# zuds-survey/zuds-pipeline

Hardware: AMD Instinct MI355X
Metric: Mpix/s resample->coadd->subtract, 3072x3072 frames (higher is better)
Workload: dtype f32; 1 GPU; configs[1]+[2]: 32x 3072x3072 TPV frames/GPU, mesh background + weight rescale + Lanczos-3 resample + WEIGHTED coadd (+ AND mask coadd, int16 masks); then 1 science frame/GPU: align ref, hotpants 3x3 regions x 10x10 stamps, r=10, ko=4, subtract; frames_per_gpu=32, size=3072, mask_dtype=int16, combine=WEIGHTED, subtract=True

## Files before the change

### zuds-pipeline_amd/csrc/hotpants.hip

```cpp
#include "hp_dev.h"
#include <sched.h>
#include "chol_diag.h"

static __device__ __forceinline__ void hp_zero_words(int* __restrict__ zero0, int nzero0, int* __restrict__ zero1, int nzero1) {
    if (blockIdx.x != 0) return;
    if (zero0) for (int k = threadIdx.x; k < nzero0; k += blockDim.x) zero0[k] = 0;
    if (zero1) for (int k = threadIdx.x; k < nzero1; k += blockDim.x) zero1[k] = 0;
}
__global__ void k_hp_valid(const float* __restrict__ sci, const float* __restrict__ ref,
                           const uint8_t* __restrict__ bpm, int64_t n, float il, float iu,
                           float tl, float tu, uint8_t* __restrict__ bad,
                           const double* __restrict__ lim, double nsig,
                           int* __restrict__ zero0 = nullptr, int nzero0 = 0,
                           int* __restrict__ zero1 = nullptr, int nzero1 = 0) {
    int64_t p = (int64_t)blockIdx.x * blockDim.x + threadIdx.x;
    hp_zero_words(zero0, nzero0, zero1, nzero1);
    if (lim) {
        il = (float)(lim[0] - nsig * lim[1]);
        tl = (float)(lim[3] - nsig * lim[4]);
    }
    if (p >= n) return;
    float s = sci[p], t = ref[p];
    bool ok = (s == s) && (t == t) && fabsf(s) < 3e38f && fabsf(t) < 3e38f;
    ok = ok && s >= il && s <= iu && t >= tl && t <= tu;
// ... 367 lines not shown
#define GR_PITCH 34

#define GR_SPLIT 8
template <int NT, int R0, int C0, int R1, int C1, int R2, int C2>
static __device__ __forceinline__ void hp_gram_ktile(const double* L, int li, int lk, double4_t (&acc)[3]) {
#pragma unroll
    for (int kk = 0; kk < GR_KT / 4; ++kk) {
        const double* Lk = L + li * GR_PITCH + 4 * kk + lk;
        acc[0] = __builtin_amdgcn_mfma_f64_16x16x4f64(Lk[16 * R0 * GR_PITCH], Lk[16 * C0 * GR_PITCH], acc[0], 0, 0, 0);
        if (NT > 1) acc[1] = __builtin_amdgcn_mfma_f64_16x16x4f64(Lk[16 * R1 * GR_PITCH], Lk[16 * C1 * GR_PITCH], acc[1], 0, 0, 0);
        if (NT > 2) acc[2] = __builtin_amdgcn_mfma_f64_16x16x4f64(Lk[16 * R2 * GR_PITCH], Lk[16 * C2 * GR_PITCH], acc[2], 0, 0, 0);
    }
}
template <int R, int C>
static __device__ __forceinline__ void hp_gram_store(double* Gc, int li, int lk, const double4_t& a) {
#pragma unroll
    for (int rg = 0; rg < 4; ++rg) {
        Gc[(size_t)(16 * R + lk + 4 * rg) * HP_MAXX + 16 * C + li] = a[rg];
        if (R != C) Gc[(size_t)(16 * C + li) * HP_MAXX + 16 * R + lk + 4 * rg] = a[rg];
    }
}
#define GR_DEAL(sel, F) \
    switch (sel) { \
        case 0: F(3, 3, 0, 3, 1, 3, 2) break; \
        case 1: F(3, 2, 0, 2, 1, 2, 2) break; \
        case 2: F(2, 1, 0, 1, 1, 0, 0) break; \
        default: F(2, 0, 0, 3, 3, 0, 0) break; \
    }
static __device__ __forceinline__ void hp_gram_body(const hp_plan& P, const double* __restrict__ X,
                                                 const int* __restrict__ need,
                                                 const int* __restrict__ active,
                                                 double* __restrict__ Gp, const int* __restrict__ guard,
                                                 const int* __restrict__ list) {
    if (guard && *guard == 0) return;
    __shared__ double L[HP_MAXX * GR_PITCH];
    const int tid = threadIdx.x;
    const int ncl = list ? list[0] : (int)gridDim.x;
#pragma unroll 1
    for (int ci = blockIdx.x; ci < ncl; ci += gridDim.x) {
    const int cell = list ? list[1 + ci] : ci;
    __syncthreads();
    if (!need[cell] || active[cell] < 0) continue;
    const double* Xc = X + (size_t)cell * P.nX * P.npixp;
    const int wave = tid >> 6, lane = tid & 63;
    const int li = lane & 15, lk = lane >> 4;
    const int sel = __builtin_amdgcn_readfirstlane((wave + blockIdx.x + blockIdx.y) & 3);
    const int ntile = P.npixp / GR_KT;
    const int per = (ntile + GR_SPLIT - 1) / GR_SPLIT;
    const int kbeg = blockIdx.y * per * GR_KT, kend = min((int)(blockIdx.y + 1) * per, ntile) * GR_KT;
    double4_t acc[3];
#pragma unroll
    for (int c = 0; c < 3; ++c) acc[c] = (double4_t){0.0, 0.0, 0.0, 0.0};
    constexpr int GR_LD = HP_MAXX * GR_KT / 256;
    double nxt[GR_LD];
    auto fetch = [&](int k0) {
#pragma unroll
        for (int q = 0; q < GR_LD; ++q) {
            const int e = tid + 256 * q, row = e >> 5, col = e & 31;
            nxt[q] = row < P.nX ? Xc[(size_t)row * P.npixp + k0 + col] : 0.0;
        }
    };
    if (kbeg < kend) fetch(kbeg);
    for (int k0 = kbeg; k0 < kend; k0 += GR_KT) {
        __syncthreads();
#pragma unroll
        for (int q = 0; q < GR_LD; ++q) {
            const int e = tid + 256 * q, row = e >> 5, col = e & 31;
            L[row * GR_PITCH + col] = nxt[q];
        }
        __syncthreads();
        if (k0 + GR_KT < kend) fetch(k0 + GR_KT);
#define GR_STEP(NT, R0, C0, R1, C1, R2, C2) hp_gram_ktile<NT, R0, C0, R1, C1, R2, C2>(L, li, lk, acc);
        GR_DEAL(sel, GR_STEP)
#undef GR_STEP
    }
    double* Gc = Gp + ((size_t)cell * GR_SPLIT + blockIdx.y) * HP_MAXX * HP_MAXX;
#define GR_OUT(NT, R0, C0, R1, C1, R2, C2) { \
        hp_gram_store<R0, C0>(Gc, li, lk, acc[0]); \
        if (NT > 1) hp_gram_store<R1, C1>(Gc, li, lk, acc[1]); \
        if (NT > 2) hp_gram_store<R2, C2>(Gc, li, lk, acc[2]); }
    GR_DEAL(sel, GR_OUT)
#undef GR_OUT
    }
}
#undef GR_DEAL

#define GS_THREADS 1024
static __device__ __forceinline__ void hp_gram_sum_body(const double* __restrict__ Gp,
                                                     const int* __restrict__ need,
                                                     const int* __restrict__ active,
                                                     double* __restrict__ G, const int* __restrict__ guard,
                                                     double* __restrict__ Gold, const int* __restrict__ list) {
    if (guard && *guard == 0) return;
    const int ncl = list ? list[0] : (int)gridDim.x;
    constexpr int NE = HP_MAXX * HP_MAXX / GS_THREADS;
#pragma unroll 1
    for (int ci = blockIdx.x; ci < ncl; ci += gridDim.x) {
        const int cell = list ? list[1 + ci] : ci;
        if (!need[cell] || active[cell] < 0) continue;
        const double* src = Gp + (size_t)cell * GR_SPLIT * HP_MAXX * HP_MAXX;
        double* dst = G + (size_t)cell * HP_MAXX * HP_MAXX;
        double* old = Gold ? Gold + (size_t)cell * HP_MAXX * HP_MAXX : nullptr;
        double part[NE][GR_SPLIT], prev[NE];
#pragma unroll
        for (int q = 0; q < NE; ++q) {
            const int e = threadIdx.x + GS_THREADS * q;
#pragma unroll
            for (int sl = 0; sl < GR_SPLIT; ++sl) part[q][sl] = src[(size_t)sl * HP_MAXX * HP_MAXX + e];
            prev[q] = old ? dst[e] : 0.0;
        }
#pragma unroll
        for (int q = 0; q < NE; ++q) {
            const int e = threadIdx.x + GS_THREADS * q;
            double v = 0.0;
#pragma unroll
            for (int sl = 0; sl < GR_SPLIT; ++sl) v += part[q][sl];
            if (old) old[e] = prev[q];
            dst[e] = v;
        }
    }
}

__device__ inline void col_decode(const hp_plan& P, int c, int* n, int* p) {
    if (c == 0) { *n = 0; *p = -1; return; }
    int k = c - 1;
    if (k < (P.nc - 1) * P.nkp) { *n = 1 + k / P.nkp; *p = k % P.nkp; return; }
    *n = P.nc + (k - (P.nc - 1) * P.nkp);
    *p = -1;
}

__global__ __launch_bounds__(256) void k_hp_build(const hp_plan P, const double* __restrict__ G,
                                                  const double* __restrict__ phi,
// ... 1509 lines not shown
        }
        diag_put(c, dnext[0]);
        if (c + CBC_COLS < CH_NB * CH_NB) diag_put(c + CBC_COLS, dnext[1]);
        __syncthreads();
        if (c < k0n) {
            double acc = 0.0;
#pragma unroll
            for (int m = 0; m < CH_NB; ++m) acc += a[m] * xc[m];
            yc -= acc;
        }
#pragma unroll
        for (int m = 0; m < CH_NB; ++m) a[m] = (c < k0n) ? A[(size_t)(k0n + m) * lda + c] : 0.0;
        if (kb > 1) {
            dnext[0] = diag_elem(k0n - CH_NB, CH_NB, c);
            if (c + CBC_COLS < CH_NB * CH_NB) dnext[1] = diag_elem(k0n - CH_NB, CH_NB, c + CBC_COLS);
        }
        __syncthreads();
    }
    if (c < min(CH_NB, n)) yc = xs[(nblk - 1) & 1][c];
    if (c < n) xall[(size_t)blockIdx.x * n + c] = yc / dall[(size_t)blockIdx.x * n + c];
}

static __device__ __forceinline__ void hp_merit_body(const hp_plan& P, const double* __restrict__ G,
                                                 const double* __restrict__ phi,
                                                 const double* __restrict__ vbar,
                                                 const int* __restrict__ active,
                                                 const double* __restrict__ xsol,
                                                 double* __restrict__ merit, const int* __restrict__ guard,
                                                 int* __restrict__ needlist) {
    if (guard && *guard == 0) return;
    __shared__ double c[HP_MAXX];
    const int cell = blockIdx.x, lane = threadIdx.x;
    if (needlist && cell == 0 && lane == 0) needlist[0] = 0;
    if (active[cell] < 0) { if (lane == 0) merit[cell] = -1.0; return; }
    const int reg = cell / P.ncellr;
    const double* x = xsol + (size_t)reg * P.nunk;
    const double* ph = phi + (size_t)cell * P.nkp;
    const double* Gc = G + (size_t)cell * HP_MAXX * HP_MAXX;
    if (lane < P.nE) {
        double v;
        if (lane == 0) v = x[0];
        else if (lane < P.nc) {
            v = 0.0;
            for (int p = 0; p < P.nkp; ++p) v += x[1 + (lane - 1) * P.nkp + p] * ph[p];
        } else v = x[1 + (P.nc - 1) * P.nkp + (lane - P.nc)];
        c[lane] = v;
    }
    __syncthreads();
    double part = 0.0;
    if (lane < P.nE) {
        double q = 0.0;
        for (int m = 0; m < P.nE; ++m) q += Gc[lane * HP_MAXX + m] * c[m];
        part = c[lane] * (q - 2.0 * Gc[lane * HP_MAXX + P.nE]);
    }
    part = wave_sum_d(part);
    if (lane == 0) merit[cell] = (Gc[P.nE * HP_MAXX + P.nE] + part) / (P.npix * vbar[cell]);
}

#define HP_RFLAG_TMO (1 << 30)
#define HP_RFLAG_DONE 0x80000000u
struct hp_sig {
    int* done;
    unsigned long long* host;
    unsigned seq;
};
static __device__ __forceinline__ void hp_round_signal(const hp_sig& sg, int* round_flag, int nblocks) {
    if (!sg.host) return;
    __threadfence();
    __syncthreads();
    if (threadIdx.x == 0 && atomicAdd(sg.done, 1) == nblocks - 1) {
        const unsigned v = (unsigned)atomicAdd(round_flag, 0);
        __threadfence_system();
        __hip_atomic_store(sg.host, ((unsigned long long)sg.seq << 32) | v | HP_RFLAG_DONE, __ATOMIC_RELEASE,
                           __HIP_MEMORY_SCOPE_SYSTEM);
    }
}
__global__ __launch_bounds__(256) void k_hp_reject(const hp_plan P, const double* __restrict__ merit,
                                                   const int2* __restrict__ centres,
                                                   int* __restrict__ active, int* __restrict__ need,
                                                   int* __restrict__ chg, int* __restrict__ nrej,
                                                   double* __restrict__ stats, const int* __restrict__ guard, int* __restrict__ round_flag,
                                                   int* __restrict__ needlist, const int* __restrict__ tmo = nullptr,
                                                   const hp_sig sig = hp_sig{nullptr, nullptr, 0u}) {
    if (guard && *guard == 0) {
        hp_round_signal(sig, round_flag, gridDim.x);
        return;
    }
    __shared__ double red[4];
    const int reg = blockIdx.x, tid = threadIdx.x;
    double m = 0.0, s = 0.0;
    for (int pass = 0; pass < 4; ++pass) {
        double s0 = 0, s1 = 0;
        for (int k = tid; k < P.ncellr; k += 256) {
            double v = merit[reg * P.ncellr + k];
            if (active[reg * P.ncellr + k] < 0) continue;
            if (pass == 0 || fabs(v - m) <= 3.0 * s) { s0 += 1.0; s1 += v; }
        }
        s0 = block_sum256(s0, red);
        s1 = block_sum256(s1, red);
        if (s0 < 1.0) break;
        double mn = s1 / s0, s2 = 0;
        for (int k = tid; k < P.ncellr; k += 256) {
            double v = merit[reg * P.ncellr + k];
            if (active[reg * P.ncellr + k] < 0) continue;
            if (pass == 0 || fabs(v - m) <= 3.0 * s) s2 += (v - mn) * (v - mn);
        }
        s2 = block_sum256(s2, red);
        m = mn;
        s = sqrt(s2 / s0);
    }
    const double lim = m + P.ks * s;
    double cnt = 0, msum = 0, used = 0;
    for (int k = tid; k < P.ncellr; k += 256) {
        const int cell = reg * P.ncellr + k;
        int a = active[cell];
        need[cell] = 0;
        chg[cell] = 0;
        if (a < 0) continue;
        double v = merit[cell];
        used += 1.0;
        msum += v;
        if (v > lim) {
            cnt += 1.0;
            a += 1;
            if (a >= P.nss || centres[cell * P.nss + a].x < 0) a = -1;
            else {
                need[cell] = 1;
                if (needlist) needlist[1 + atomicAdd(&needlist[0], 1)] = cell;
            }
            active[cell] = a;
            chg[cell] = 1;
        }
    }
    cnt = block_sum256(cnt, red);
    msum = block_sum256(msum, red);
    used = block_sum256(used, red);
    if (tid == 0) {
        nrej[reg] = (int)cnt;
        if (cnt > 0) atomicAdd(round_flag, (int)cnt);
        if (tmo && tmo[reg]) atomicOr(round_flag, HP_RFLAG_TMO);
        stats[reg * 2 + 0] = used > 0 ? msum / used : 0.0;
        stats[reg * 2 + 1] = used;
    }
    __syncthreads();
    if (tid == 0) {
        int* list = chg + P.ncell + reg * (P.ncellr + 1);
        int k = 0;
        for (int c = 0; c < P.ncellr; ++c)
            if (chg[reg * P.ncellr + c]) list[1 + k++] = reg * P.ncellr + c;
        list[0] = k;
    }
    hp_round_signal(sig, round_flag, gridDim.x);
}

static __device__ __forceinline__ void hp_reject_wave_body(const hp_plan& P, const double* __restrict__ merit,
                                                       const int2* __restrict__ centres,
                                                       int* __restrict__ active, int* __restrict__ need,
                                                       int* __restrict__ chg, int* __restrict__ nrej,
                                                       double* __restrict__ stats, const int* __restrict__ guard,
                                                       int* __restrict__ round_flag, int* __restrict__ needlist,
                                                       const int* __restrict__ tmo = nullptr) {
    if (guard && *guard == 0) return;
    const int reg = blockIdx.x, lane = threadIdx.x;
    double mv[4];
    int av[4];
#pragma unroll
    for (int u = 0; u < 4; ++u) {
        const int k = lane + 64 * u;
        mv[u] = k < P.ncellr ? merit[reg * P.ncellr + k] : 0.0;
        av[u] = k < P.ncellr ? active[reg * P.ncellr + k] : -1;
    }
    double m = 0.0, s = 0.0;
    for (int pass = 0; pass < 4; ++pass) {
        double s0 = 0, s1 = 0;
#pragma unroll
        for (int u = 0; u < 4; ++u)
            if (av[u] >= 0 && (pass == 0 || fabs(mv[u] - m) <= 3.0 * s)) { s0 += 1.0; s1 += mv[u]; }
        s0 = wave_sum_d(s0);
        s1 = wave_sum_d(s1);
        if (s0 < 1.0) break;
        const double mn = s1 / s0;
        double s2 = 0;
#pragma unroll
        for (int u = 0; u < 4; ++u)
            if (av[u] >= 0 && (pass == 0 || fabs(mv[u] - m) <= 3.0 * s)) s2 += (mv[u] - mn) * (mv[u] - mn);
        s2 = wave_sum_d(s2);
        m = mn;
        s = sqrt(s2 / s0);
    }
    const double lim = m + P.ks * s;
    double cnt = 0, msum = 0, used = 0;
    unsigned long long chm[4];
#pragma unroll
    for (int u = 0; u < 4; ++u) {
        const int k = lane + 64 * u;
        bool changed = false;
        if (k < P.ncellr) {
            const int cell = reg * P.ncellr + k;
            int a = av[u];
            int nd = 0;
            if (a >= 0) {
                used += 1.0;
                msum += mv[u];
                if (mv[u] > lim) {
                    cnt += 1.0;
                    a += 1;
                    if (a >= P.nss || centres[cell * P.nss + a].x < 0) a = -1;
                    else nd = 1;
                    active[cell] = a;
                    changed = true;
                }
            }
            need[cell] = nd;
            chg[cell] = changed ? 1 : 0;
            if (nd && needlist) needlist[1 + atomicAdd(&needlist[0], 1)] = cell;
        }
        chm[u] = __ballot(changed);
    }
    cnt = wave_sum_d(cnt);
    msum = wave_sum_d(msum);
    used = wave_sum_d(used);
    if (lane == 0) {
        nrej[reg] = (int)cnt;
        if (cnt > 0) atomicAdd(round_flag, (int)cnt);
        if (tmo && tmo[reg]) atomicOr(round_flag, HP_RFLAG_TMO);
        stats[reg * 2 + 0] = used > 0 ? msum / used : 0.0;
        stats[reg * 2 + 1] = used;
    }
    int* list = chg + P.ncell + reg * (P.ncellr + 1);
    int base = 0;
#pragma unroll
    for (int u = 0; u < 4; ++u) {
        const unsigned long long bm = chm[u];
        if (bm >> lane & 1ull)
            list[1 + base + __popcll(bm & ((1ull << lane) - 1ull))] = reg * P.ncellr + lane + 64 * u;
        base += __popcll(bm);
    }
    if (lane == 0) list[0] = base;
}

__global__ void k_hp_init_active(const hp_plan P, const int2* __restrict__ centres,
                                 int* __restrict__ active, int* __restrict__ need,
                                 int* __restrict__ ntotal) {
    int cell = blockIdx.x * blockDim.x + threadIdx.x;
    if (cell >= P.ncell) return;
    bool has = centres[cell * P.nss].x >= 0;
    active[cell] = has ? 0 : -1;
    need[cell] = has ? 1 : 0;
    if (has) atomicAdd(&ntotal[cell / P.ncellr], 1);
}

__global__ __launch_bounds__(256) void k_hp_gram(const hp_plan P, const double* __restrict__ X,
                                                 const int* __restrict__ need, const int* __restrict__ active,
                                                 double* __restrict__ Gp, const int* __restrict__ guard,
                                                 const int* __restrict__ list) {
    hp_gram_body(P, X, need, active, Gp, guard, list);
}
__global__ __launch_bounds__(256) void k_hp_gram_b(const hp_plan P, const hp_job* __restrict__ jobs, int round) {
    const hp_job& J = jobs[blockIdx.z];
    hp_gram_body(P, J.X, J.need, J.active, J.Gp, HPJ_GUARD(J, round), round > 1 ? J.needlist : nullptr);
}

__global__ __launch_bounds__(GS_THREADS) void k_hp_gram_sum(const double* __restrict__ Gp, const int* __restrict__ need,
                                                     const int* __restrict__ active, double* __restrict__ G,
                                                     const int* __restrict__ guard, double* __restrict__ Gold,
                                                     const int* __restrict__ list) {
    hp_gram_sum_body(Gp, need, active, G, guard, Gold, list);
}
__global__ __launch_bounds__(GS_THREADS) void k_hp_gram_sum_b(const hp_job* __restrict__ jobs, int round) {
    const hp_job& J = jobs[blockIdx.z];
    hp_gram_sum_body(J.Gp, J.need, J.active, J.G, HPJ_GUARD(J, round), J.Gold, round > 1 ? J.needlist : nullptr);
}

__global__ __launch_bounds__(256) void k_hp_build_blk(const hp_plan P, const double* __restrict__ G,
                                                      const double* __restrict__ phi, const int* __restrict__ active,
                                                      const int* __restrict__ chg, int sign, double* __restrict__ A,
                                                      double* __restrict__ rhs, const int* __restrict__ guard,
                                                      unsigned* __restrict__ zero = nullptr, int nzero = 0,
                                                      const double* __restrict__ Gold = nullptr,
                                                      const double* __restrict__ phiold = nullptr,
                                                      const int* __restrict__ need = nullptr) {
    __shared__ double sh[BB_LDS];
    if (guard && *guard == 0) return;
    const int reg = blockIdx.z;
    if (sign == 2) {
        hp_update_blk_body(reg, blockIdx.x * HBB_PAIRS, P, G, phi, active, chg, A, rhs, zero, nzero, Gold, phiold, need, sh);
        return;
    }
    const int npair = P.nE * (P.nE + 1) / 2;
#pragma unroll 1
    for (int pair = blockIdx.x * HBB_PAIRS; pair < min((int)(blockIdx.x + 1) * HBB_PAIRS, npair); ++pair)
        hp_build_blk_body(reg, pair, P, G, phi, active, A, rhs, zero, nzero, sh);
}
__global__ __launch_bounds__(256) void k_hp_build_blk_b(const hp_plan P, const hp_job* __restrict__ jobs, int round) {
    __shared__ double sh[BB_LDS];
    const hp_job& J = jobs[blockIdx.y];
    const int* guard = HPJ_GUARD(J, round);
    if (guard && *guard == 0) return;
    const int reg = blockIdx.z;
    if (round > 1) {
        hp_update_blk_body(reg, blockIdx.x * HBB_PAIRS, P, J.G, J.phi, J.active, J.chg, J.A0, J.rhs0, nullptr, 0, J.Gold,
                           J.phiold, J.need, sh);
        return;
    }
// ... 360 lines not shown
    info->status = (nsolved == nreg ? 0 : ZM_HP_UNSOLVED);
    info->nunsolved = nreg - nsolved;
    info->retries = retries;
}

extern "C" int zm_subtract_dev(zm_ctx* ctx, const float* sci, const float* sci_rms, const float* ref,
                               const float* ref_rms, const uint8_t* bpm, int nx, int ny,
                               const zm_hp_params* hp, float* out_diff, float* out_rms,
                               zm_hp_info* info) {
    ZM_CHECK(ctx && sci && sci_rms && ref && ref_rms && hp && out_diff && out_rms,
             "zm_subtract_dev: null argument");
    ZM_CHECK(nx > 0 && ny > 0, "zm_subtract_dev: empty image");
    ZM_HIP(hipSetDevice(ctx->device));
    hp_plan P;
    std::vector<double> filt, basis;
    ZM_TRY(make_plan(hp, nx, ny, &P, &filt, &basis));
    ZM_CHECK(nx > 2 * P.hw + 1 && ny > 2 * P.hw + 1, "zm_subtract_dev: image smaller than a substamp");
    const int64_t np = (int64_t)nx * ny;
    hipStream_t st = ctx->stream;

    uint8_t *bad = nullptr, *tmp8 = nullptr, *dirty = nullptr, *outbad = nullptr;
    ZM_TRY(ctx->get("hp_bad", np, (void**)&bad));
    ZM_TRY(ctx->get("hp_tmp8", np, (void**)&tmp8));
    ZM_TRY(ctx->get("hp_dirty", np, (void**)&dirty));
    ZM_TRY(ctx->get("hp_outbad", np, (void**)&outbad));
    int2* centres = nullptr;
    int *active = nullptr, *need = nullptr, *ibuf = nullptr;
    double *X = nullptr, *G = nullptr, *phi = nullptr, *vbar = nullptr, *A = nullptr, *rhs = nullptr,
           *dsc = nullptr, *merit = nullptr, *stats = nullptr, *d_filt = nullptr;
    ZM_TRY(ctx->get("hp_centres", sizeof(int2) * P.ncell * P.nss, (void**)&centres));
    ZM_TRY(ctx->get("hp_active", sizeof(int) * P.ncell, (void**)&active));
    ZM_TRY(ctx->get("hp_need", sizeof(int) * P.ncell, (void**)&need));
    int* needlist = nullptr;
    ZM_TRY(ctx->get("hp_needlist", sizeof(int) * ((size_t)P.ncell + 1), (void**)&needlist));
    int* chg = nullptr;
    ZM_TRY(ctx->get("hp_chg", sizeof(int) * (2 * (size_t)P.ncell + P.nreg), (void**)&chg));
    constexpr int HP_NIBUF = 4 * HP_MAXREG + 4;
    constexpr size_t HP_SUMBYTES = sizeof(int) * HP_NIBUF + sizeof(double) * 3 * HP_MAXREG;
    static_assert((sizeof(int) * HP_NIBUF) % 8 == 0, "the statistics behind the counters are doubles");
    char* sumbuf = nullptr;
    ZM_TRY(ctx->get("hp_summary", HP_SUMBYTES, (void**)&sumbuf));
    ibuf = reinterpret_cast<int*>(sumbuf);
    int *nrej = ibuf, *ntotal = ibuf + HP_MAXREG, *fail = ibuf + 2 * HP_MAXREG, *nmasked = ibuf + 3 * HP_MAXREG;
    int* tmo = ibuf + 3 * HP_MAXREG + 4;
    unsigned* cbar = nullptr;
    ZM_TRY(ctx->get("hp_cbar", sizeof(unsigned) * CF_BAR_STRIDE * HP_MAXREG, (void**)&cbar));
    double* cdg = nullptr;
    ZM_TRY(ctx->get("hp_cdg", sizeof(double) * 4 * CH_NB * (CH_NB + 1) * HP_MAXREG, (void**)&cdg));
    ZM_TRY(ctx->get("hp_X", sizeof(double) * (size_t)P.ncell * P.nX * P.npixp, (void**)&X));
    ZM_TRY(ctx->get("hp_G", sizeof(double) * (size_t)P.ncell * HP_MAXX * HP_MAXX, (void**)&G));
    double* Gp = nullptr;
    ZM_TRY(ctx->get("hp_Gp", sizeof(double) * (size_t)P.ncell * GR_SPLIT * HP_MAXX * HP_MAXX, (void**)&Gp));
    ZM_TRY(ctx->get("hp_phi", sizeof(double) * (size_t)P.ncell * P.nkp, (void**)&phi));
    double *Gold = nullptr, *phiold = nullptr;
    ZM_TRY(ctx->get("hp_Gold", sizeof(double) * (size_t)P.ncell * HP_MAXX * HP_MAXX, (void**)&Gold));
    ZM_TRY(ctx->get("hp_phiold", sizeof(double) * (size_t)P.ncell * P.nkp, (void**)&phiold));
    ZM_TRY(ctx->get("hp_vbar", sizeof(double) * P.ncell, (void**)&vbar));
    const int lda = (P.nunk + 15) & ~15;
    ZM_TRY(ctx->get("hp_A", sizeof(double) * (size_t)P.nreg * (P.nunk + 1) * lda, (void**)&A));
    ZM_TRY(ctx->get("hp_rhs", sizeof(double) * (size_t)P.nreg * P.nunk, (void**)&rhs));
    double *A0 = nullptr, *rhs0 = nullptr;
    ZM_TRY(ctx->get("hp_A0", sizeof(double) * (size_t)P.nreg * (P.nunk + 1) * P.nunk, (void**)&A0));
    ZM_TRY(ctx->get("hp_rhs0", sizeof(double) * (size_t)P.nreg * P.nunk, (void**)&rhs0));
    ZM_TRY(ctx->get("hp_dsc", sizeof(double) * (size_t)P.nreg * P.nunk, (void**)&dsc));
    ZM_TRY(ctx->get("hp_merit", sizeof(double) * P.ncell, (void**)&merit));
    stats = reinterpret_cast<double*>(sumbuf + sizeof(int) * HP_NIBUF);
    double* x0sum = stats + 2 * HP_MAXREG;
// ... 35 lines not shown

    int* h_rflags = nullptr;
    hipEvent_t* evs = nullptr;
    ZM_TRY(ctx->get_pinned("hp_rflags_h", sizeof(int) * 16, (void**)&h_rflags));
    ZM_TRY(zm_get_sync_events(ctx, 3, &evs));
    if (attempt > 0) ZM_HIP(hipMemsetAsync(rflags, 0, sizeof(int) * 32, st));
    if (!ctx->hp_sig_h) {
        ZM_HIP(hipHostMalloc((void**)&ctx->hp_sig_h, sizeof(unsigned long long) * 16, hipHostMallocCoherent | hipHostMallocMapped));
        memset(ctx->hp_sig_h, 0, sizeof(unsigned long long) * 16);
        ZM_HIP(hipHostGetDevicePointer((void**)&ctx->hp_sig_d, ctx->hp_sig_h, 0));
    }
    static const bool sig_off = ZM_DEVENV("ZM_HP_SIGNAL") && ZM_DEVENV("ZM_HP_SIGNAL")[0] == '0';
    const unsigned seq = ++ctx->hp_seq;
    auto enqueue_round = [&](const int rounds) -> int {
        const int* guard = rounds > 1 ? rflags + (rounds - 1) : nullptr;
        const int ncl_grid = std::min(P.ncell, 48);
        if (rounds > 1) {
            zm_scope_timer t(ctx, "hp_solve");
            int nt = zm_div_up(P.nunk, 16);
            if (P.nkp > 16)
                hipLaunchKernelGGL(k_hp_build, dim3(nt, nt, P.nreg), b256, 0, st, P, G, phi, active, chg, -1, A0, rhs0, guard);
        }
        {
            zm_scope_timer t(ctx, "hp_vectors");
            ZM_TRY(zm_hp_launch_vectors(ctx, st, P, hvc, rounds, ncl_grid, hv_gx, sci, ref, sci_rms, ref_rms, d_filt, centres, active,
                                        need, X, phi, vbar, guard, phiold, needlist, hv_w0g));
            ZM_HIP(hipGetLastError());
        }
        {
            zm_scope_timer t(ctx, "hp_gram");
            hipLaunchKernelGGL(k_hp_gram, dim3(rounds == 1 ? P.ncell : ncl_grid, GR_SPLIT), b256, 0, st, P, X, need, active, Gp, guard,
                               rounds == 1 ? nullptr : needlist);
            hipLaunchKernelGGL(k_hp_gram_sum, dim3(rounds == 1 ? P.ncell : ncl_grid), dim3(GS_THREADS), 0, st, Gp, need, active, G, guard, Gold,
                               rounds == 1 ? nullptr : needlist);
            ZM_HIP(hipGetLastError());
        }
        {
            zm_scope_timer t(ctx, "hp_solve");
            int nt = zm_div_up(P.nunk, 16);
            const char* form_env = getenv("ZM_CHOL_FORM");
            bool tp = safe || ctx->share >= 2 || fitting.shared();
            if (form_env && !strcmp(form_env, "tp")) tp = true;
            if (form_env && (!strcmp(form_env, "lat") || !strcmp(form_env, "df")) && !safe) tp = false;
            if (!ctx->hp_wg_cap) {
                int occ = 0, ncu = 0;
                ZM_HIP(hipOccupancyMaxActiveBlocksPerMultiprocessor(&occ, (const void*)k_chol_fused, 256, 0));
                ZM_HIP(hipDeviceGetAttribute(&ncu, hipDeviceAttributeMultiprocessorCount, ctx->device));
                ctx->hp_wg_cap = std::max(1, std::min(occ, 1) * (ncu - ncu / 16));
                if (ZM_DEVENV("ZM_CHOL_PROF")) fprintf(stderr, "chol: occupancy %d x %d CUs\n", occ, ncu);
            }
            const int wg_cap = ctx->hp_wg_cap / std::max(ctx->share, 1);
            const int W = std::max(2, std::min(68, wg_cap / P.nreg));
            const int nunk = P.nunk;
            static const bool want_prof = ZM_DEVENV("ZM_CHOL_PROF") && atoi(ZM_DEVENV("ZM_CHOL_PROF")) != 0;
            const bool want_df = !tp && !(form_env && !strcmp(form_env, "lat")) && 2 * P.nreg <= wg_cap && W <= 128;
            const int ndff = hp_df_nflags(P.nunk);
            unsigned* dff = nullptr;
            double* dfdg = nullptr;
            int* dftiles = nullptr;
            bool df = want_df;
            if (df) {
                constexpr int TW = 1 + 2 * DF_MAXT;
                int* htl = nullptr;
                ZM_TRY(ctx->get_pinned("hp_dftiles_h", sizeof(int) * (3 + 128 * TW), (void**)&htl));
                ZM_TRY(ctx->get("hp_dftiles", sizeof(int) * 128 * TW, (void**)&dftiles));
                constexpr int DF_MAGIC = 0x64663031;
                const bool known = htl[2] == DF_MAGIC && htl[1] == W && (htl[0] == nunk || htl[0] == -nunk - 1);
// ... 256 lines not shown
    ZM_CHECK(ctx && jobs && njobs >= 1 && njobs <= ZM_SUB_BATCH_MAX, "zm_subtract_batch_dev: 1 .. %d jobs", ZM_SUB_BATCH_MAX);
    ZM_CHECK(nx > 0 && ny > 0, "zm_subtract_batch_dev: empty image");
    ZM_HIP(hipSetDevice(ctx->device));
    std::vector<hp_plan> Pj(njobs);
    std::vector<double> filt, basis, filt_j, basis_j;
    for (int j = 0; j < njobs; ++j) {
        const zm_sub_job& jb = jobs[j];
        ZM_CHECK(jb.sci && jb.sci_rms && jb.ref && jb.ref_rms && jb.params && jb.out_diff && jb.out_rms,
                 "zm_subtract_batch_dev: null argument in job %d", j);
        ZM_TRY(make_plan(jb.params, nx, ny, &Pj[j], j == 0 ? &filt : &filt_j, j == 0 ? &basis : &basis_j));
        ZM_CHECK(j == 0 || (hp_plans_agree(Pj[0], Pj[j]) && filt_j == filt),
                 "zm_subtract_batch_dev: job %d asks for a different fit (half widths, basis, orders, regions, stamps or "
                 "thresholds) than job 0 - batch jobs of one configuration", j);
    }
    const hp_plan& P = Pj[0];
    ZM_CHECK(nx > 2 * P.hw + 1 && ny > 2 * P.hw + 1, "zm_subtract_batch_dev: image smaller than a substamp");
    if (P.nkp > 15 || P.nunk > CBC_COLS || P.ncellr > 256 || njobs == 1 || P.hwk > 15 || hp_vectors_cfg(P.pw, P.sw, P.npix).big) {
        for (int j = 0; j < njobs; ++j)
            ZM_TRY(zm_subtract_dev(ctx, jobs[j].sci, jobs[j].sci_rms, jobs[j].ref, jobs[j].ref_rms, jobs[j].bpm, nx, ny,
                                   jobs[j].params, jobs[j].out_diff, jobs[j].out_rms, infos ? &infos[j] : nullptr));
        return 0;
    }
    const int64_t np = (int64_t)nx * ny;
    hipStream_t st = ctx->stream;
    const int lda = (P.nunk + 15) & ~15;
    const int ldt = (P.nunk + 1 + 15) & ~15;
    constexpr int HP_NIBUF = 4 * HP_MAXREG + 4;

    size_t off = 0;
    auto take = [&](size_t bytes) { const size_t o = off; off += (bytes + 255) & ~(size_t)255; return o; };
    const size_t o_bad = take(np), o_dirty = take(np), o_outbad = take(np);
    const size_t o_centres = take(sizeof(int2) * P.ncell * P.nss);
    const size_t o_active = take(sizeof(int) * P.ncell), o_need = take(sizeof(int) * P.ncell);
    const size_t o_needlist = take(sizeof(int) * ((size_t)P.ncell + 1));
    const size_t o_chg = take(sizeof(int) * (2 * (size_t)P.ncell + P.nreg));
    const size_t o_X = take(sizeof(double) * (size_t)P.ncell * P.nX * P.npixp);
    const size_t o_G = take(sizeof(double) * (size_t)P.ncell * HP_MAXX * HP_MAXX);
    const size_t o_Gp = take(sizeof(double) * (size_t)P.ncell * GR_SPLIT * HP_MAXX * HP_MAXX);
    const size_t o_Gold = take(sizeof(double) * (size_t)P.ncell * HP_MAXX * HP_MAXX);
    const size_t o_phi = take(sizeof(double) * (size_t)P.ncell * P.nkp);
    const size_t o_phiold = take(sizeof(double) * (size_t)P.ncell * P.nkp);
    const size_t o_vbar = take(sizeof(double) * P.ncell);
    const size_t o_A = take(sizeof(double) * (size_t)P.nreg * (P.nunk + 1) * lda);
    const size_t o_AT = take(sizeof(double) * (size_t)P.nreg * P.nunk * ldt);
    const size_t o_rhs = take(sizeof(double) * (size_t)P.nreg * P.nunk);
    const size_t o_A0 = take(sizeof(double) * (size_t)P.nreg * (P.nunk + 1) * P.nunk);
    const size_t o_rhs0 = take(sizeof(double) * (size_t)P.nreg * P.nunk);
    const size_t o_dsc = take(sizeof(double) * (size_t)P.nreg * P.nunk);
    const size_t o_merit = take(sizeof(double) * P.ncell);
    const size_t o_smask = take(sizeof(unsigned long long));
    const size_t slab = off;
    char* base = nullptr;
    ZM_TRY(ctx->get("hpb_slab", slab * (size_t)njobs, (void**)&base));
    uint8_t* tmp8 = nullptr;
    ZM_TRY(ctx->get("hp_tmp8", np, (void**)&tmp8));
    int *ibuf_all = nullptr, *rflags_all = nullptr, *h_rflags = nullptr;
    ZM_TRY(ctx->get("hpb_ibuf", sizeof(int) * HP_NIBUF * (size_t)njobs, (void**)&ibuf_all));
    ZM_TRY(ctx->get("hpb_rflags", sizeof(int) * 16 * (size_t)njobs, (void**)&rflags_all));
    double* sum_all = nullptr;
    ZM_TRY(ctx->get("hpb_sum", sizeof(double) * 3 * HP_MAXREG * (size_t)njobs, (void**)&sum_all));
    ZM_TRY(ctx->get_pinned("hpb_rflags_h", sizeof(int) * 32 * (size_t)njobs, (void**)&h_rflags));
    hp_job *h_jobs = nullptr, *d_jobs = nullptr;
    ZM_TRY(ctx->get_pinned("hpb_jobs_h", sizeof(hp_job) * (size_t)njobs * 9, (void**)&h_jobs));
    ZM_TRY(ctx->get("hpb_jobs", sizeof(hp_job) * (size_t)njobs * 9, (void**)&d_jobs));
    double* d_filt = nullptr;
    ZM_TRY(ctx->get("hp_filt", sizeof(double) * filt.size(), (void**)&d_filt));
    hipEvent_t* evs = nullptr;
// ... 25 lines not shown
    ZM_HIP(hipMemcpyAsync(d_jobs, h_jobs, sizeof(hp_job) * (size_t)njobs, hipMemcpyHostToDevice, st));
    ZM_HIP(hipMemsetAsync(ibuf_all, 0, sizeof(int) * HP_NIBUF * (size_t)njobs, st));
    ZM_HIP(hipMemsetAsync(rflags_all, 0, sizeof(int) * 16 * (size_t)njobs, st));

    for (int j = 0; j < njobs; ++j) {
        char* sb = base + slab * (size_t)j;
        const hp_job& J = h_jobs[j];
        ZM_TRY(hp_launch_masks(ctx, Pj[j], jobs[j].params, jobs[j].sci, jobs[j].ref, jobs[j].bpm, (uint8_t*)(sb + o_bad), tmp8,
                               (uint8_t*)(sb + o_dirty), (uint8_t*)(sb + o_outbad)));
        ZM_TRY(hp_launch_cells(ctx, Pj[j], jobs[j].ref, (uint8_t*)(sb + o_bad), (uint8_t*)(sb + o_dirty), J.centres, J.active,
                               J.need, HPJ_NTOTAL(J)));
    }

    const size_t vsh = hp_vectors_cfg(P.pw, P.sw, P.npix).shmem;
    const dim3 b256(256);
    std::vector<int> live(njobs);
    for (int j = 0; j < njobs; ++j) live[j] = j;
    auto enqueue_round = [&](const int round) -> int {
        zm_scope_timer t(ctx, "hpb_fit");
        const hp_job* d_tab = d_jobs;
        unsigned NJ = (unsigned)njobs;
        if (round >= 3) {
            hp_job* h_tab = h_jobs + (size_t)njobs * (round - 1);
            for (size_t k = 0; k < live.size(); ++k) h_tab[k] = h_jobs[live[k]];
            NJ = (unsigned)live.size();
            if (NJ == 0) return 0;
            d_tab = d_jobs + (size_t)njobs * (round - 1);
            ZM_HIP(hipMemcpyAsync((void*)d_tab, h_tab, sizeof(hp_job) * NJ, hipMemcpyHostToDevice, st));
        }
        const int ncl_grid = std::min(P.ncell, 12);
        const unsigned gcells = round == 1 ? P.ncell : ncl_grid;
        ZM_TRY(zm_hp_launch_vectors_b(ctx, st, P, vsh, gcells, NJ, d_tab, d_filt, round));
        hipLaunchKernelGGL(k_hp_gram_b, dim3(gcells, GR_SPLIT, NJ), b256, 0, st, P, d_tab, round);
        hipLaunchKernelGGL(k_hp_gram_sum_b, dim3(gcells, 1, NJ), dim3(GS_THREADS), 0, st, d_tab, round);
        static const bool build_scalar = ZM_DEVENV("ZM_BUILD_FORM") && !strcmp(ZM_DEVENV("ZM_BUILD_FORM"), "scalar");
        if (round == 1 && !build_scalar)
            hipLaunchKernelGGL(k_hp_build_mfma_b, dim3(zm_div_up(P.nE * (P.nE + 1) / 2, 4), P.nreg, NJ), b256, 0, st, P, d_tab);
        else
            hipLaunchKernelGGL(k_hp_build_blk_b, dim3(zm_div_up(P.nE * (P.nE + 1) / 2, HBB_PAIRS), NJ, P.nreg), b256, 0, st, P, d_tab, round);
        hipLaunchKernelGGL(k_hp_diag_b, dim3(zm_div_up(P.nunk, 256), P.nreg, NJ), b256, 0, st, P.nunk, d_tab, round);
        hipLaunchKernelGGL(k_hp_scale_b, dim3(zm_div_up(P.nunk, HSB_ROWS), P.nreg * NJ), b256, 0, st, P.nunk, lda, P.nreg,
                           d_tab, round, P.ncell, P.ncellr);
        hipLaunchKernelGGL(k_chol_tp_b, dim3(P.nreg, 1, NJ), dim3(CT_THREADS), 0, st, P.nunk, lda, ldt, d_tab, round, P.ncell, P.ncellr);
        hipLaunchKernelGGL(k_chol_back_cols_b, dim3(P.nreg, 1, NJ), dim3(CBC_THREADS), 0, st, P.nunk, lda, d_tab, round, P.ncell, P.ncellr);
        hipLaunchKernelGGL(k_hp_merit_b, dim3(P.ncell, 1, NJ), dim3(64), 0, st, P, d_tab, round);
        hipLaunchKernelGGL(k_hp_reject_wave_b, dim3(P.nreg, 1, NJ), dim3(64), 0, st, P, d_tab, round);
        ZM_HIP(hipGetLastError());
        ZM_HIP(hipMemcpyAsync(h_rflags + 16 * (size_t)njobs * (round & 1), rflags_all, sizeof(int) * 16 * (size_t)njobs,
                              hipMemcpyDeviceToHost, st));
        ZM_HIP(hipEventRecord(evs[1 + (round & 1)], st));
        return 0;
    };
    auto enqueue_apply = [&](const int j) -> int {
        zm_scope_timer t(ctx, "hp_apply");
        char* sb = base + slab * (size_t)j;
        const hp_job& J = h_jobs[j];
        hipLaunchKernelGGL(k_hp_solved, dim3(1), dim3(64), 0, ctx->stream, P.nreg, P.nunk, J.stats, HPJ_FAIL(J), HPJ_TMO(J),
                           J.rhs, J.smask, J.stats + 2 * HP_MAXREG);
        ZM_TRY(zm_hp_launch_apply(ctx, Pj[j], J.smask, jobs[j].sci, jobs[j].ref, jobs[j].sci_rms, jobs[j].ref_rms,
                                  (uint8_t*)(sb + o_outbad), d_filt, J.rhs, jobs[j].out_diff, jobs[j].out_rms, HPJ_NMASKED(J)));
        if (jobs[j].params->flag_mask_dev)
            ZM_TRY(zm_mask_flag_dev(ctx, jobs[j].params->flag_mask_dev, jobs[j].out_diff, 1e-30f, jobs[j].params->flag_bit, np));
        return 0;
    };
    static const bool apply_beside = !(ZM_DEVENV("ZM_BATCH_APPLY") && !strcmp(ZM_DEVENV("ZM_BATCH_APPLY"), "after"));
    struct stream_swap {
        zm_ctx* c; hipStream_t keep;
// ... 137 lines not shown
```

### zuds-pipeline_amd/csrc/hp_dev.h

```cpp
#pragma once
#include <algorithm>
#include <atomic>
#include <cmath>

#include "zm_internal.h"

#define HP_MAXX 64
#define HP_MAXPOLY 28
#define HP_MAXNSS 8
#define HP_MAXREG 64
#define CF_BAR_STRIDE 32
#define HP_MAXF1 32
#define HP_RIDGE 1e-10

struct hp_plan {
    int nx, ny, hwk, hwss, hw, step, sw, npix, npixp, pw;
    int nc, nbg, nE, nX, nkp, nunk, ko, bgo;
    int nrx, nry, nsx, nsy, nss, nreg, ncellr, ncell, nf1;
    int normalize;
    double tu, tl, iu, il, ft, ks;
    float fi, fin;
    int rx0[HP_MAXREG], rx1[HP_MAXREG], ry0[HP_MAXREG], ry1[HP_MAXREG];
    int tfx[HP_MAXX], tfy[HP_MAXX], tsub0[HP_MAXX];
    double tscale[HP_MAXX];
// ... 45 lines not shown
#define HV_SPLIT_FEW 16

#define HV_THREADS 512
#define HP_MAX_HWK 20
#define HP_MAX_HWSS 60
struct hv_cfg { bool big; bool w0_global; int cw; size_t shmem; };
static inline hv_cfg hp_vectors_cfg(int pw, int sw, int npix) {
    const size_t lim = 160 * 1024, patch = sizeof(float) * (size_t)pw * (pw + 8) + 16;
    const size_t fast = sizeof(double) * ((size_t)(pw + 8) * sw + npix + 8) + patch;
    if (fast <= lim) return {false, false, sw, fast};
    const size_t full = sizeof(double) * ((size_t)(pw + 8) * sw + 8) + patch;
    if (full <= lim) return {true, true, sw, full};
    if (patch + sizeof(double) * 8 + sizeof(double) * (size_t)(pw + 8) * 8 > lim) return {true, true, 0, 0};
    int cw = (int)((lim - patch - sizeof(double) * 8) / (sizeof(double) * (size_t)(pw + 8)));
    cw &= ~7;
    return {true, true, cw, sizeof(double) * ((size_t)(pw + 8) * cw + 8) + patch};
}

struct hp_job {
    const float *sci, *ref, *srms, *trms;
    int2* centres;
    int *active, *need, *needlist, *chg, *ibuf, *rflags;
    double *X, *G, *Gp, *Gold, *phi, *phiold, *vbar, *A, *AT, *rhs, *A0, *rhs0, *dsc, *merit, *stats;
    unsigned long long* smask;
};
#define HPJ_NREJ(J) ((J).ibuf)
#define HPJ_NTOTAL(J) ((J).ibuf + HP_MAXREG)
#define HPJ_FAIL(J) ((J).ibuf + 2 * HP_MAXREG)
#define HPJ_NMASKED(J) ((J).ibuf + 3 * HP_MAXREG)
#define HPJ_TMO(J) ((J).ibuf + 3 * HP_MAXREG + 4)
#define HPJ_GUARD(J, round) ((round) > 1 ? (J).rflags + ((round) - 1) : nullptr)
#define HPJ_REGION_IDLE(J, round, reg, ncell, ncellr) ((round) > 1 && (J).chg[(ncell) + (reg) * ((ncellr) + 1)] == 0)

int zm_hp_launch_vectors(zm_ctx* ctx, hipStream_t st, const hp_plan& P, const hv_cfg& hvc, int rounds, int ncl_grid, int hv_gx,
                         const float* sci, const float* ref, const float* sci_rms, const float* ref_rms, const double* filt,
                         const int2* centres, const int* active, const int* need, double* X, double* phi, double* vbar,
                         const int* guard, double* phiold, const int* needlist, double* hv_w0g);
int zm_hp_launch_vectors_b(zm_ctx* ctx, hipStream_t st, const hp_plan& P, size_t vsh, unsigned gcells, unsigned njobs,
                           const hp_job* d_tab, const double* filt, int round);
int zm_hp_launch_apply(zm_ctx* ctx, const hp_plan& P, const unsigned long long* solved_mask, const float* sci,
                       const float* ref, const float* srms, const float* trms, const uint8_t* outbad,
                       const double* filt, const double* xsol, float* diff, float* noise, int* nmasked);
```

### zuds-pipeline_amd/csrc/hp_vectors.hip

```cpp
#include "hp_dev.h"

static __device__ __forceinline__ void hv_pin(double (&a)[8]) {
    asm volatile("" : "+v"(a[0]), "+v"(a[1]), "+v"(a[2]), "+v"(a[3]), "+v"(a[4]), "+v"(a[5]), "+v"(a[6]), "+v"(a[7]));
}
static __device__ __forceinline__ void hv_pin(double (&a)[5]) {
    asm volatile("" : "+v"(a[0]), "+v"(a[1]), "+v"(a[2]), "+v"(a[3]), "+v"(a[4]));
}

#define HV_RY 5
static __device__ __forceinline__ int hv_rows_y(int cwe, int sw) {
    return (cwe * ((sw + HV_R - 1) / HV_R) > HV_THREADS / 2 && cwe * ((sw + HV_RY - 1) / HV_RY) <= HV_THREADS) ? HV_RY : HV_R;
}

template <int HWK, int R, bool PIN>
static __device__ __forceinline__ void hv_ypass(int tid, int cwe, int c0, int sw, const double* xp, int cw,
                                             const double* __restrict__ fyv, double sc, bool sub0, bool first, bool mine,
                                             double* w0, char* Xn) {
    constexpr int STEP = 2 * HWK + 1, WIN = R + 2 * HWK;
    const unsigned rowb = (unsigned)sw * (unsigned)sizeof(double);
    const unsigned cwb = (unsigned)cw * (unsigned)sizeof(double);
    const int nstrip = (sw + R - 1) / R;
    for (int e = tid; e < cwe * nstrip; e += HV_THREADS) {
        const int s = e / cwe, jl = e - s * cwe, j = c0 + jl;
        const int i0 = s * R;
// ... 20 lines not shown
        double wsub[R];
#pragma unroll
        for (int q = 0; q < R; ++q) wsub[q] = 0.0;
        if (sub0) {
            const int klast = (sw - 1) * sw + j;
#pragma unroll
            for (int q = 0; q < R; ++q) wsub[q] = w0[min(k0 + q * sw, klast)];
        }
#pragma unroll
        for (int q = 0; q < R; ++q) {
            const double v = acc[q] * sc - wsub[q];
            if (q < nv) {
                if (first) w0[k0 + q * sw] = v;
                if (mine) *reinterpret_cast<double*>(Xn + ((unsigned)k0 * (unsigned)sizeof(double) + q * rowb)) = v;
            }
        }
    }
}

template <int HWK, bool BIG = false>
static __device__ __forceinline__ void hp_vectors_body(const hp_plan& P, const float* __restrict__ sci,
                                                    const float* __restrict__ ref,
                                                    const float* __restrict__ srms,
                                                    const float* __restrict__ trms,
                                                    const double* __restrict__ filt,
                                                    const int2* __restrict__ centres,
                                                    const int* __restrict__ active,
                                                    const int* __restrict__ need,
                                                    double* __restrict__ X,
                                                    double* __restrict__ phi,
                                                    double* __restrict__ vbar, const int* __restrict__ guard,
                                                    double* __restrict__ phiold, const int* __restrict__ list,
                                                    int special, int cwarg = 0, double* __restrict__ w0g = nullptr) {
    if (guard && *guard == 0) return;
    extern __shared__ double hp_smem[];
    constexpr int STEP = 2 * HWK + 1;
    constexpr int WIN = HV_R + 2 * HWK;
    const int tid = threadIdx.x;
    const int part = blockIdx.y, nparts = gridDim.y;
    const int ncl = list ? list[0] : (BIG ? P.ncell : (int)gridDim.x);
#pragma unroll 1
    for (int ci = blockIdx.x; ci < ncl; ci += gridDim.x) {
    const int cell = list ? list[1 + ci] : ci;
    __syncthreads();
    if (!need[cell]) continue;
    const int act = active[cell];
    if (act < 0) continue;
    const int2 cc = centres[cell * P.nss + act];
    const int r = cell / P.ncellr;
    const int pw = P.pw, sw = P.sw, hwss = P.hwss;
    const bool only_special = special && part == 0;
    const int fpart = special ? part - 1 : part, fparts = special ? nparts - 1 : nparts;
    const int pp = pw + HV_R;
    const int cw = BIG ? cwarg : P.sw;
    double* xp = hp_smem;
    double* w0 = (BIG && w0g) ? w0g + ((size_t)blockIdx.y * gridDim.x + blockIdx.x) * (size_t)P.npix
                              : xp + (size_t)(pw + HV_R) * cw;
    double* red = (BIG && w0g) ? xp + (size_t)(pw + HV_R) * cw : w0 + P.npix;
    float* patch = reinterpret_cast<float*>(red + 8);
    for (int k0 = tid; !only_special && k0 < pw * pw; k0 += HV_THREADS * 10) {
        float t[10];
#pragma unroll
        for (int u = 0; u < 10; ++u) {
            const int k = k0 + HV_THREADS * u;
            const int yy = k / pw, xx = k - yy * pw;
            t[u] = (k < pw * pw) ? ref[(size_t)(cc.y - P.hw + yy) * P.nx + (cc.x - P.hw + xx)] : 0.f;
        }
#pragma unroll
        for (int u = 0; u < 10; ++u) {
            const int k = k0 + HV_THREADS * u;
            const int yy = k / pw, xx = k - yy * pw;
            if (k < pw * pw) patch[yy * pp + xx] = t[u];
        }
    }
#pragma clang loop vectorize(disable) interleave(disable) unroll(disable)
    for (int k = tid; k < pw * HV_R; k += HV_THREADS) patch[(k / HV_R) * pp + pw + k % HV_R] = 0.f;
#pragma clang loop vectorize(disable) interleave(disable) unroll(disable)
    for (int k = tid; k < HV_R * cw; k += HV_THREADS) xp[(size_t)pw * cw + k] = 0.0;
    const double xc = P.rx0[r] + 0.5 * (P.rx1[r] - P.rx0[r]), hx = 0.5 * (P.rx1[r] - P.rx0[r]);
    const double yc = P.ry0[r] + 0.5 * (P.ry1[r] - P.ry0[r]), hy = 0.5 * (P.ry1[r] - P.ry0[r]);
    double* Xc = X + (size_t)cell * P.nX * P.npixp;
// ... 184 lines not shown
```

Baseline: 50870 Mpix/s.

## Store full work records in the needlist and prefetch them in persistent loops

Result: no change. 50980 Mpix/s, median of 5 (+0.2%).

```diff
diff --git a/zuds-pipeline_amd/csrc/hotpants.hip b/zuds-pipeline_amd/csrc/hotpants.hip
--- a/zuds-pipeline_amd/csrc/hotpants.hip
+++ b/zuds-pipeline_amd/csrc/hotpants.hip
@@ -423,15 +423,24 @@
                                                  const int* __restrict__ active,
                                                  double* __restrict__ Gp, const int* __restrict__ guard,
                                                  const int* __restrict__ list) {
-    if (guard && *guard == 0) return;
+    int gv = 1, ncl = (int)gridDim.x;
+    int4 rec = make_int4(0, 0, 0, 0);
+    int nslots = P.ncell;
+    asm volatile("" : "+s"(nslots));
+    if (list) hp_work_head(guard, list, nslots, gv, ncl, rec);
+    else if (guard) gv = *guard;
+    if (gv == 0) return;
     __shared__ double L[HP_MAXX * GR_PITCH];
     const int tid = threadIdx.x;
-    const int ncl = list ? list[0] : (int)gridDim.x;
 #pragma unroll 1
     for (int ci = blockIdx.x; ci < ncl; ci += gridDim.x) {
-    const int cell = list ? list[1 + ci] : ci;
+    int cell = ci;
+    if (list) {
+        cell = __builtin_amdgcn_readfirstlane(rec.x);
+        rec = hp_work_rec(list, min(ci + (int)gridDim.x, ncl - 1));
+    }
     __syncthreads();
-    if (!need[cell] || active[cell] < 0) continue;
+    if (!list && (!need[cell] || active[cell] < 0)) continue;
     const double* Xc = X + (size_t)cell * P.nX * P.npixp;
     const int wave = tid >> 6, lane = tid & 63;
     const int li = lane & 15, lk = lane >> 4;
@@ -481,14 +490,22 @@
                                                      const int* __restrict__ need,
                                                      const int* __restrict__ active,
                                                      double* __restrict__ G, const int* __restrict__ guard,
-                                                     double* __restrict__ Gold, const int* __restrict__ list) {
-    if (guard && *guard == 0) return;
-    const int ncl = list ? list[0] : (int)gridDim.x;
+                                                     double* __restrict__ Gold, const int* __restrict__ list,
+                                                     int ncell) {
+    int gv = 1, ncl = (int)gridDim.x;
+    int4 rec = make_int4(0, 0, 0, 0);
+    asm volatile("" : "+s"(ncell));
+    if (list) hp_work_head(guard, list, ncell, gv, ncl, rec);
+    else if (guard) gv = *guard;
+    if (gv == 0) return;
     constexpr int NE = HP_MAXX * HP_MAXX / GS_THREADS;
 #pragma unroll 1
     for (int ci = blockIdx.x; ci < ncl; ci += gridDim.x) {
-        const int cell = list ? list[1 + ci] : ci;
-        if (!need[cell] || active[cell] < 0) continue;
+        int cell = ci;
+        if (list) {
+            cell = __builtin_amdgcn_readfirstlane(rec.x);
+            rec = hp_work_rec(list, min(ci + (int)gridDim.x, ncl - 1));
+        } else if (!need[cell] || active[cell] < 0) continue;
         const double* src = Gp + (size_t)cell * GR_SPLIT * HP_MAXX * HP_MAXX;
         double* dst = G + (size_t)cell * HP_MAXX * HP_MAXX;
         double* old = Gold ? Gold + (size_t)cell * HP_MAXX * HP_MAXX : nullptr;
@@ -2064,20 +2081,23 @@
     __shared__ double c[HP_MAXX];
     const int cell = blockIdx.x, lane = threadIdx.x;
     if (needlist && cell == 0 && lane == 0) needlist[0] = 0;
-    if (active[cell] < 0) { if (lane == 0) merit[cell] = -1.0; return; }
+    int act = active[cell];
+    double vb = vbar[cell];
     const int reg = cell / P.ncellr;
     const double* x = xsol + (size_t)reg * P.nunk;
     const double* ph = phi + (size_t)cell * P.nkp;
     const double* Gc = G + (size_t)cell * HP_MAXX * HP_MAXX;
+    double v = 0.0;
     if (lane < P.nE) {
-        double v;
         if (lane == 0) v = x[0];
         else if (lane < P.nc) {
-            v = 0.0;
             for (int p = 0; p < P.nkp; ++p) v += x[1 + (lane - 1) * P.nkp + p] * ph[p];
         } else v = x[1 + (P.nc - 1) * P.nkp + (lane - P.nc)];
-        c[lane] = v;
-    }
+    }
+    act = __builtin_amdgcn_readfirstlane(act);
+    asm volatile("" : "+s"(act), "+v"(vb), "+v"(v));
+    if (act < 0) { if (lane == 0) merit[cell] = -1.0; return; }
+    if (lane < P.nE) c[lane] = v;
     __syncthreads();
     double part = 0.0;
     if (lane < P.nE) {
@@ -2086,7 +2106,7 @@
         part = c[lane] * (q - 2.0 * Gc[lane * HP_MAXX + P.nE]);
     }
     part = wave_sum_d(part);
-    if (lane == 0) merit[cell] = (Gc[P.nE * HP_MAXX + P.nE] + part) / (P.npix * vbar[cell]);
+    if (lane == 0) merit[cell] = (Gc[P.nE * HP_MAXX + P.nE] + part) / (P.npix * vb);
 }
 
 #define HP_RFLAG_TMO (1 << 30)
@@ -2146,19 +2166,20 @@
     for (int k = tid; k < P.ncellr; k += 256) {
         const int cell = reg * P.ncellr + k;
         int a = active[cell];
+        const double v = merit[cell];
+        const int2 cn = centres[cell * P.nss + min(max(a + 1, 0), P.nss - 1)];
         need[cell] = 0;
         chg[cell] = 0;
         if (a < 0) continue;
-        double v = merit[cell];
         used += 1.0;
         msum += v;
         if (v > lim) {
             cnt += 1.0;
             a += 1;
-            if (a >= P.nss || centres[cell * P.nss + a].x < 0) a = -1;
+            if (a >= P.nss || cn.x < 0) a = -1;
             else {
                 need[cell] = 1;
-                if (needlist) needlist[1 + atomicAdd(&needlist[0], 1)] = cell;
+                if (needlist) hp_work_put(needlist, cell, a, cn);
             }
             active[cell] = a;
             chg[cell] = 1;
@@ -2201,6 +2222,12 @@
         const int k = lane + 64 * u;
         mv[u] = k < P.ncellr ? merit[reg * P.ncellr + k] : 0.0;
         av[u] = k < P.ncellr ? active[reg * P.ncellr + k] : -1;
+    }
+    int2 cn[4];
+#pragma unroll
+    for (int u = 0; u < 4; ++u) {
+        const int cell = reg * P.ncellr + min(lane + 64 * u, P.ncellr - 1);
+        cn[u] = centres[cell * P.nss + min(max(av[u] + 1, 0), P.nss - 1)];
     }
     double m = 0.0, s = 0.0;
     for (int pass = 0; pass < 4; ++pass) {
@@ -2237,7 +2264,7 @@
                 if (mv[u] > lim) {
                     cnt += 1.0;
                     a += 1;
-                    if (a >= P.nss || centres[cell * P.nss + a].x < 0) a = -1;
+                    if (a >= P.nss || cn[u].x < 0) a = -1;
                     else nd = 1;
                     active[cell] = a;
                     changed = true;
@@ -2245,7 +2272,7 @@
             }
             need[cell] = nd;
             chg[cell] = changed ? 1 : 0;
-            if (nd && needlist) needlist[1 + atomicAdd(&needlist[0], 1)] = cell;
+            if (nd && needlist) hp_work_put(needlist, cell, a, cn[u]);
         }
         chm[u] = __ballot(changed);
     }
@@ -2296,12 +2323,12 @@
 __global__ __launch_bounds__(GS_THREADS) void k_hp_gram_sum(const double* __restrict__ Gp, const int* __restrict__ need,
                                                      const int* __restrict__ active, double* __restrict__ G,
                                                      const int* __restrict__ guard, double* __restrict__ Gold,
-                                                     const int* __restrict__ list) {
-    hp_gram_sum_body(Gp, need, active, G, guard, Gold, list);
-}
-__global__ __launch_bounds__(GS_THREADS) void k_hp_gram_sum_b(const hp_job* __restrict__ jobs, int round) {
+                                                     const int* __restrict__ list, int ncell) {
+    hp_gram_sum_body(Gp, need, active, G, guard, Gold, list, ncell);
+}
+__global__ __launch_bounds__(GS_THREADS) void k_hp_gram_sum_b(const hp_job* __restrict__ jobs, int round, int ncell) {
     const hp_job& J = jobs[blockIdx.z];
-    hp_gram_sum_body(J.Gp, J.need, J.active, J.G, HPJ_GUARD(J, round), J.Gold, round > 1 ? J.needlist : nullptr);
+    hp_gram_sum_body(J.Gp, J.need, J.active, J.G, HPJ_GUARD(J, round), J.Gold, round > 1 ? J.needlist : nullptr, ncell);
 }
 
 __global__ __launch_bounds__(256) void k_hp_build_blk(const hp_plan P, const double* __restrict__ G,
@@ -2728,7 +2755,7 @@
     ZM_TRY(ctx->get("hp_active", sizeof(int) * P.ncell, (void**)&active));
     ZM_TRY(ctx->get("hp_need", sizeof(int) * P.ncell, (void**)&need));
     int* needlist = nullptr;
-    ZM_TRY(ctx->get("hp_needlist", sizeof(int) * ((size_t)P.ncell + 1), (void**)&needlist));
+    ZM_TRY(ctx->get("hp_needlist", HP_WORK_BYTES(P.ncell), (void**)&needlist));
     int* chg = nullptr;
     ZM_TRY(ctx->get("hp_chg", sizeof(int) * (2 * (size_t)P.ncell + P.nreg), (void**)&chg));
     constexpr int HP_NIBUF = 4 * HP_MAXREG + 4;
@@ -2830,7 +2857,7 @@
             hipLaunchKernelGGL(k_hp_gram, dim3(rounds == 1 ? P.ncell : ncl_grid, GR_SPLIT), b256, 0, st, P, X, need, active, Gp, guard,
                                rounds == 1 ? nullptr : needlist);
             hipLaunchKernelGGL(k_hp_gram_sum, dim3(rounds == 1 ? P.ncell : ncl_grid), dim3(GS_THREADS), 0, st, Gp, need, active, G, guard, Gold,
-                               rounds == 1 ? nullptr : needlist);
+                               rounds == 1 ? nullptr : needlist, P.ncell);
             ZM_HIP(hipGetLastError());
         }
         {
@@ -3153,7 +3180,7 @@
     const size_t o_bad = take(np), o_dirty = take(np), o_outbad = take(np);
     const size_t o_centres = take(sizeof(int2) * P.ncell * P.nss);
     const size_t o_active = take(sizeof(int) * P.ncell), o_need = take(sizeof(int) * P.ncell);
-    const size_t o_needlist = take(sizeof(int) * ((size_t)P.ncell + 1));
+    const size_t o_needlist = take(HP_WORK_BYTES(P.ncell));
     const size_t o_chg = take(sizeof(int) * (2 * (size_t)P.ncell + P.nreg));
     const size_t o_X = take(sizeof(double) * (size_t)P.ncell * P.nX * P.npixp);
     const size_t o_G = take(sizeof(double) * (size_t)P.ncell * HP_MAXX * HP_MAXX);
@@ -3245,7 +3272,7 @@
         const unsigned gcells = round == 1 ? P.ncell : ncl_grid;
         ZM_TRY(zm_hp_launch_vectors_b(ctx, st, P, vsh, gcells, NJ, d_tab, d_filt, round));
         hipLaunchKernelGGL(k_hp_gram_b, dim3(gcells, GR_SPLIT, NJ), b256, 0, st, P, d_tab, round);
-        hipLaunchKernelGGL(k_hp_gram_sum_b, dim3(gcells, 1, NJ), dim3(GS_THREADS), 0, st, d_tab, round);
+        hipLaunchKernelGGL(k_hp_gram_sum_b, dim3(gcells, 1, NJ), dim3(GS_THREADS), 0, st, d_tab, round, P.ncell);
         static const bool build_scalar = ZM_DEVENV("ZM_BUILD_FORM") && !strcmp(ZM_DEVENV("ZM_BUILD_FORM"), "scalar");
         if (round == 1 && !build_scalar)
             hipLaunchKernelGGL(k_hp_build_mfma_b, dim3(zm_div_up(P.nE * (P.nE + 1) / 2, 4), P.nreg, NJ), b256, 0, st, P, d_tab);
diff --git a/zuds-pipeline_amd/csrc/hp_dev.h b/zuds-pipeline_amd/csrc/hp_dev.h
--- a/zuds-pipeline_amd/csrc/hp_dev.h
+++ b/zuds-pipeline_amd/csrc/hp_dev.h
@@ -101,6 +101,31 @@
 #define HPJ_GUARD(J, round) ((round) > 1 ? (J).rflags + ((round) - 1) : nullptr)
 #define HPJ_REGION_IDLE(J, round, reg, ncell, ncellr) ((round) > 1 && (J).chg[(ncell) + (reg) * ((ncellr) + 1)] == 0)
 
+#define HP_WORK_BYTES(ncell) (sizeof(int4) * ((size_t)(ncell) + 1))
+static __device__ __forceinline__ int4 hp_work_rec(const int* __restrict__ list, int k) {
+    return reinterpret_cast<const int4*>(list)[1 + k];
+}
+static __device__ __forceinline__ void hp_work_put(int* __restrict__ list, int cell, int act, int2 c) {
+    const int k = atomicAdd(&list[0], 1);
+    reinterpret_cast<int4*>(list)[1 + k] = make_int4(cell, act, c.x, c.y);
+}
+static __device__ __forceinline__ void hp_work_pin(int& guard, int& count, int4& rec) {
+    guard = __builtin_amdgcn_readfirstlane(guard);
+    count = __builtin_amdgcn_readfirstlane(count);
+    rec.x = __builtin_amdgcn_readfirstlane(rec.x);
+    rec.y = __builtin_amdgcn_readfirstlane(rec.y);
+    rec.z = __builtin_amdgcn_readfirstlane(rec.z);
+    rec.w = __builtin_amdgcn_readfirstlane(rec.w);
+    asm volatile("" : "+s"(guard), "+s"(count), "+s"(rec.x), "+s"(rec.y), "+s"(rec.z), "+s"(rec.w));
+}
+static __device__ __forceinline__ void hp_work_head(const int* __restrict__ guard, const int* __restrict__ list, int ncell,
+                                                  int& gv, int& count, int4& rec) {
+    gv = *guard;
+    count = list[0];
+    rec = hp_work_rec(list, min((int)blockIdx.x, ncell - 1));
+    hp_work_pin(gv, count, rec);
+}
+
 int zm_hp_launch_vectors(zm_ctx* ctx, hipStream_t st, const hp_plan& P, const hv_cfg& hvc, int rounds, int ncl_grid, int hv_gx,
                          const float* sci, const float* ref, const float* sci_rms, const float* ref_rms, const double* filt,
                          const int2* centres, const int* active, const int* need, double* X, double* phi, double* vbar,
diff --git a/zuds-pipeline_amd/csrc/hp_vectors.hip b/zuds-pipeline_amd/csrc/hp_vectors.hip
--- a/zuds-pipeline_amd/csrc/hp_vectors.hip
+++ b/zuds-pipeline_amd/csrc/hp_vectors.hip
@@ -76,21 +76,34 @@
                                                     double* __restrict__ vbar, const int* __restrict__ guard,
                                                     double* __restrict__ phiold, const int* __restrict__ list,
                                                     int special, int cwarg = 0, double* __restrict__ w0g = nullptr) {
-    if (guard && *guard == 0) return;
+    int gv = 1, ncl = BIG ? P.ncell : (int)gridDim.x;
+    int4 rec = make_int4(0, 0, 0, 0);
+    int nslots = P.ncell;
+    asm volatile("" : "+s"(nslots));
+    if (list) hp_work_head(guard, list, nslots, gv, ncl, rec);
+    else if (guard) gv = *guard;
+    if (gv == 0) return;
     extern __shared__ double hp_smem[];
     constexpr int STEP = 2 * HWK + 1;
     constexpr int WIN = HV_R + 2 * HWK;
     const int tid = threadIdx.x;
     const int part = blockIdx.y, nparts = gridDim.y;
-    const int ncl = list ? list[0] : (BIG ? P.ncell : (int)gridDim.x);
 #pragma unroll 1
     for (int ci = blockIdx.x; ci < ncl; ci += gridDim.x) {
-    const int cell = list ? list[1 + ci] : ci;
+    int cell = ci;
+    int2 cc;
+    if (list) {
+        cell = __builtin_amdgcn_readfirstlane(rec.x);
+        cc = make_int2(__builtin_amdgcn_readfirstlane(rec.z), __builtin_amdgcn_readfirstlane(rec.w));
+        rec = hp_work_rec(list, min(ci + (int)gridDim.x, ncl - 1));
+    }
     __syncthreads();
-    if (!need[cell]) continue;
-    const int act = active[cell];
-    if (act < 0) continue;
-    const int2 cc = centres[cell * P.nss + act];
+    if (!list) {
+        if (!need[cell]) continue;
+        const int act = active[cell];
+        if (act < 0) continue;
+        cc = centres[cell * P.nss + act];
+    }
     const int r = cell / P.ncellr;
     const int pw = P.pw, sw = P.sw, hwss = P.hwss;
     const bool only_special = special && part == 0;
```
